# QData/FastSK

Measured on AMD Instinct MI355X. Metric: gkm kernel build: mismatch-combos/s, higher is better.
Workload: dtype u4 count planes (v_dot8_u32_u4), u32 register sums, u64 triangle (plain stores on the first pass over reset rows, else atomics); 1 GPU; config5: synthetic DNA 100000 x 300 bp, g=12 m=8 exact, 495 combos; n_seq=100000, seq_len=300, g=12, m=8, combos=495, parallelism=single GPU

## Files before the change

### fastsk_amd/csrc/fsk_engine_dense_shift.hip

```cpp
#include "fsk_engine_internal.h"
#include "fsk_kernels_dense_shift.h"

#include <map>

using namespace fsk_detail;

namespace fsk {

#define FSK_DMA_SHIFT 1
#define FSK_DMA_KERNEL k_dense_tile_shift
#define FSK_DMA_COMPACT 0
#include "fsk_tile_kernel_dma.inc"
#undef FSK_DMA_KERNEL
#undef FSK_DMA_COMPACT
#undef FSK_DMA_SHIFT

}

namespace fsk_detail {

bool dense_shift_plan(fsk_engine* e, const int32_t* combos, int n, u64 by_overflow, uint32_t max_chain) {
    ShiftPlan& p = e->shift;
    if (!(p.by_overflow == by_overflow && p.max_chain == max_chain && (int)p.combos.size() == n && std::equal(combos, combos + n, p.combos.begin()))) {
        p = ShiftPlan();
        p.combos.assign(combos, combos + n);
        p.by_overflow = by_overflow;
        p.max_chain = max_chain;
        const int k = e->k;
        std::map<std::vector<uint8_t>, std::vector<std::pair<int, int>>> shapes;
        for (int q = 0; q < n; ++q) {
            const uint8_t* pos = &e->all_pos[(size_t)combos[q] * k];
            std::vector<uint8_t> shape(pos, pos + k);
            for (auto& x : shape) x = (uint8_t)(x - pos[0]);
            shapes[shape].push_back({(int)pos[0], q});
        }
        std::vector<std::vector<int>> chains;
        for (auto& kv : shapes) {
            auto& v = kv.second;
            std::stable_sort(v.begin(), v.end(), [](const std::pair<int, int>& a, const std::pair<int, int>& b) { return a.first < b.first; });
            for (size_t i = 0; i < v.size(); ++i) {
                if (i == 0 || v[i].first != v[i - 1].first + 1 || (max_chain != 0u && chains.back().size() >= max_chain)) chains.emplace_back();
                chains.back().push_back(v[i].second);
            }
        }
        std::stable_sort(chains.begin(), chains.end(), [](const std::vector<int>& a, const std::vector<int>& b) { return a.size() > b.size(); });
        p.n_bases = (uint32_t)chains.size();
        p.order.resize((size_t)n);
        uint32_t derived = p.n_bases;
        size_t group_begin = 0;
        for (size_t c = 0; c < chains.size(); ++c) {
            const std::vector<int>& ch = chains[c];
            const uint32_t len = (uint32_t)ch.size();
            p.order[c] = ch[0];
            if (c == 0 || chains[c - 1].size() != ch.size() || (u64)(c - group_begin) >= by_overflow) {
                p.groups.push_back(0u);
                p.groups.push_back(len);
                group_begin = c;
            }
            p.groups[p.groups.size() - 2] = (uint32_t)c + 1u;
            uint32_t lower = (uint32_t)c;
            for (uint32_t u = 1; u < len; ++u) {
                const uint32_t upper = derived++;
                p.order[upper] = ch[u];
                p.steps.push_back(upper << 16 | lower);
                p.steps.push_back(len - u);
                p.wsum += len - u;
                lower = upper;
            }
        }
    }
    return !p.steps.empty() && n <= 32768 && ((u64)2 * e->maxW + 32) * p.wsum < ((u64)1 << 31);
}

int dense_shift_edge_keys(fsk_engine* e, const uint8_t* chunk_pos, uint32_t panels_pad) {
    ShiftPlan& p = e->shift;
    const uint32_t n_steps = (uint32_t)(p.steps.size() / 2), np_seq = panels_pad * fsk::PANEL;
    FSK_HIP(e->d_shift_steps.reserve(p.steps.size()));
    FSK_HIP(e->d_edge_keys.reserve((size_t)n_steps * np_seq));
    FSK_HIP(hipMemcpyAsync(e->d_shift_steps.p, p.steps.data(), p.steps.size() * sizeof(uint32_t), hipMemcpyHostToDevice, e->stream));
    FSK_LAUNCH(fsk::k_dense_edge_keys, dim3(panels_pad, (n_steps + 3u) / 4u), dim3(256), 0, e->stream, e->view(), e->cfg.g, e->k, e->sigma, chunk_pos,
               (const uint32_t*)e->d_shift_steps.p, n_steps, np_seq, e->d_edge_keys.p);
    FSK_HIP(hipStreamSynchronize(e->stream));
    e->st.launches += 1;
    return FSK_OK;
}

int dense_shift_keymajor(fsk_engine* e, uint32_t panels_pad, int nb, uint32_t Vq8) {
    const ShiftPlan& p = e->shift;
    e->shift_packed = false;
    if (e->tune.dense_shift_packed < 0 || p.max_chain != SHIFT_PACKED_CHAIN) return FSK_OK;
    const size_t plane = (size_t)panels_pad * Vq8 * fsk::PANEL * (size_t)nb;
    const size_t n_keys = (p.steps.size() / 2) * (size_t)panels_pad * fsk::PANEL;
    const size_t want = (2 * plane + n_keys) * sizeof(uint32_t);
    const char* why = nullptr;
    if (e->tune.dense_shift_plane_kb > 0 && want > (size_t)e->tune.dense_shift_plane_kb * 1024) why = "over the dense_shift_plane_kb cap";
    const size_t grow = (std::max(plane, e->d_KM.cap) - e->d_KM.cap + std::max(plane, e->d_KMH.cap) - e->d_KMH.cap +
                         std::max(n_keys, e->d_edge_offs.cap) - e->d_edge_offs.cap) * sizeof(uint32_t);
    if (!why && grow > 0) {
        size_t free_b = 0, total_b = 0;
        if (hipMemGetInfo(&free_b, &total_b) != hipSuccess) free_b = 0;
        if (grow > free_b / 2) why = "more than half of the free device memory";
        else if (e->d_KM.reserve(plane) != hipSuccess || e->d_KMH.reserve(plane) != hipSuccess || e->d_edge_offs.reserve(n_keys) != hipSuccess) {
            (void)hipGetLastError();
            e->d_KM.release(); e->d_KMH.release(); e->d_edge_offs.release();
            why = "hipMalloc failed";
        }
    }
    if (why) {
        if (e->trace())
            fprintf(stderr, "[fsk] dense shift classes: the key-major planes (%.1f MB) do not fit, %s: k_dense_shift_fix runs the corrections\n",
                    (double)want / 1e6, why);
        return FSK_OK;
    }
    const uint32_t n_pairs = panels_pad / 2u;
    const uint32_t kgrid = (uint32_t)(((size_t)n_pairs * nb * Vq8 * 16u + 255u) / 256u);
    FSK_LAUNCH(fsk::k_dense_keymajor, dim3(kgrid), dim3(256), 0, e->stream, (const uint32_t*)e->d_C4.p, n_pairs, nb, Vq8, e->d_KM.p);
    FSK_LAUNCH(fsk::k_dense_keymajor, dim3(kgrid), dim3(256), 0, e->stream, (const uint32_t*)e->d_C4H.p, n_pairs, nb, Vq8, e->d_KMH.p);
    FSK_LAUNCH(fsk::k_dense_edge_offs, dim3((uint32_t)((n_keys + 255u) / 256u)), dim3(256), 0, e->stream, (const uint16_t*)e->d_edge_keys.p, n_keys,
               e->d_edge_offs.p);
    e->st.launches += 3;
    e->shift_packed = true;
    return FSK_OK;
}

int dense_shift_tiles(fsk_engine* e, u64 n_tiles, int nb, uint32_t Vq8, uint32_t nst, u64* K, int store, uint32_t panels_pad) {
    const ShiftPlan& p = e->shift;
    int slot0 = 0;
    for (size_t gi = 0; gi + 1 < p.groups.size(); gi += 2) {
        const int end = (int)p.groups[gi];
        FSK_LAUNCH(fsk::k_dense_tile_shift, dim3((uint32_t)n_tiles, 1), dim3(256), 0, e->stream, (const uint32_t*)e->d_C4.p, (const uint32_t*)e->d_C4H.p,
                   (const uint32_t*)e->d_rowmask.p, (const uint32_t*)e->d_tiletab.p, nb, Vq8, nst, (uint32_t)e->N, K, end - slot0, gi == 0 ? store : 0,
                   slot0, p.groups[gi + 1]);
        slot0 = end;
    }
    if (e->shift_packed) {
        FSK_LAUNCH(fsk::k_dense_shift_packed, dim3((uint32_t)n_tiles), dim3(256), 0, e->stream, (const uint32_t*)e->d_KM.p, (const uint32_t*)e->d_KMH.p,
                   (const uint32_t*)e->d_rowmask.p, (const uint32_t*)e->d_tiletab.p, (const uint32_t*)e->d_shift_steps.p, (uint32_t)(p.steps.size() / 2),
                   (const uint32_t*)e->d_edge_offs.p, panels_pad * fsk::PANEL, nb, Vq8, p.n_bases, (uint32_t)(32u * p.wsum), (uint32_t)e->N, K);
    } else {
        FSK_LAUNCH(fsk::k_dense_shift_fix, dim3((uint32_t)n_tiles), dim3(512), 0, e->stream, (const uint32_t*)e->d_C4.p, (const uint32_t*)e->d_C4H.p,
                   (const uint32_t*)e->d_rowmask.p, (const uint32_t*)e->d_tiletab.p, (const uint32_t*)e->d_shift_steps.p, (uint32_t)(p.steps.size() / 2),
                   (const uint16_t*)e->d_edge_keys.p, panels_pad * fsk::PANEL, nb, Vq8, (uint32_t)e->N, K);
    }
    e->st.launches += (int32_t)(p.groups.size() / 2);
    return FSK_OK;
}

}
```

### fastsk_amd/csrc/fsk_engine_internal.h

```cpp
#pragma once
#include "fsk_common.h"

#include <algorithm>
#include <chrono>
#include <cmath>
#include <cstdarg>
#include <cstdio>
#include <cstdlib>
#include <cstring>
#include <string>
#include <array>
#include <atomic>
#include <thread>
#include <vector>

#include <cstdint>
#include <climits>

#include "../../include/fastsk_amd.h"
#include <condition_variable>
#include <functional>
#include <memory>
#include <mutex>

struct fsk_group;

namespace fsk_detail {

#define FSK_HIP(call)                                                                          \
    do {                                                                                       \
        hipError_t _e = (call);                                                                \
        if (_e != hipSuccess) return e->fail(FSK_EDEVICE, "%s failed: %s", #call, hipGetErrorString(_e)); \
    } while (0)

template <typename T>
struct DevBuf {
    T* p = nullptr;
    size_t cap = 0;
    hipError_t reserve(size_t n) {
        if (n <= cap) return hipSuccess;
        if (p) (void)hipFree(p);
        p = nullptr;
        cap = 0;
        hipError_t r = hipMalloc((void**)&p, n * sizeof(T));
        if (r == hipSuccess) cap = n;
        return r;
    }
    void release() {
        if (p) (void)hipFree(p);
        p = nullptr;
        cap = 0;
    }
};

struct DeviceScope {
    int prev = -1, dev;
    hipError_t err = hipSuccess;
    explicit DeviceScope(int d) : dev(d) {
        if (hipGetDevice(&prev) != hipSuccess) prev = -1;
        if (prev != dev) err = hipSetDevice(dev);
    }
    ~DeviceScope() {
        if (prev >= 0 && prev != dev) (void)hipSetDevice(prev);
    }
    DeviceScope(const DeviceScope&) = delete;
    DeviceScope& operator=(const DeviceScope&) = delete;
};
#define FSK_ON_DEVICE(e)                                                                      \
    DeviceScope fsk_on_device_((e)->cfg.device);                                             \
    if (fsk_on_device_.err != hipSuccess)                                                    \
        return (e)->fail(FSK_EDEVICE, "hipSetDevice(%d) failed: %s", (e)->cfg.device, hipGetErrorString(fsk_on_device_.err))

}

using fsk_detail::DevBuf;

#define FSK_TUNING_KEYS(X)                                                                                                          \
    X(trace, 0, 0, 1, "stderr: the tuning in force, where the host time of a load and of a variance-mode call goes")                 \
    X(profile, -1, -1, 2, "fsk_config.profile from here on (-1: as the engine was created)")                                          \
    X(compact, -1, -1, 1, "dense: key compaction off / on whatever the alphabet says (-1: a rare symbol decides)")                   \
    X(compact_rare, -1, -1, 1, "dense: keys that occur from the places of the rare symbols (1) or a marking pass over every window (0)") \
    X(tile_splits, 0, 0, 4096, "dense: combo splits per tile (0: by the size of the launch)")                                        \
    X(dense_small, 0, 0, 1, "dense: 1 = a split tile launch (small N) leaves its sums as 32-bit staging blocks that k_dense_widen adds into K (0: one 64-bit atomic a cell and split — measured faster: the atomics drain under other workgroups' dot products)")                                        \
    X(dense_shift, 0, -1, 1, "dense: one weighted Gram product per chain of shifted combinations, the other members by edge lookups (fsk_engine_dense_shift.hip) — 1 = whenever the call is eligible, -1 = never (0: when eligible, tile_splits = 0 and the launch has 16384 tiles or more, the size from which a tile has one workgroup anyway)") \
    X(dense_shift_packed, 0, -1, 0, "dense, shift classes: the derived steps from key-major planes, eight cells an LDS read (k_dense_keymajor, k_dense_shift_packed; chains cut at nine members) — 0 = whenever the shift path runs and the planes fit, -1 = never: k_dense_shift_fix on the count panels") \
    X(dense_shift_plane_kb, 0, 0, (int64_t)1 << 40, "dense, shift classes: the key-major planes and offsets may take this many KiB at most (0: half of the free memory; tests: the planes do not fit)") \
    X(dense_chunk, 0, 0, 1 << 24, "dense: cap of the count kernel's staging chunk, in windows (0: none)")                             \
    X(variance_dense_slots, 1, 0, 1, "variance mode, dense: 0 = zero fill + k_welford per iteration instead of storing slot triangles") \
    X(var_slots16, 1, 0, 1, "variance mode, sparse: 0 = u32 slot triangles from the start")                                          \
    X(sparse_global, 0, 0, 1, "sparse: every += as a 64-bit atomicAdd (k_sx_emit<DIRECT>) whatever N is")                             \
    X(sparse_unpacked, 0, 0, 1, "sparse: entries in the general 8 + 4 (+ 4) byte format whatever N is")                               \
    X(sparse_pairs, 1, 0, 1, "sparse: 0 = every update word 32 bits wide (1: unit products of clean runs travel two to a word)")      \
    X(sparse_sync, 0, 0, 1, "sparse: wait for every batch's word count and size its stream exactly")                                 \
    X(sparse_hint, 1, 0, 1, "sparse: 0 = the words per record of the previous set of sequences are never kept as a hint")             \
    X(sparse_exact_lanes, 0, 0, 2, "sparse: the batches of an exact accumulate never (1) / always (2) in two lanes (0: from six batches on)") \
    X(sparse_batch_records, 0, 0, (int64_t)1 << 31, "sparse: records per batch at most (0: 2^27)")                                   \
    X(guard_cap, 0, 0, (int64_t)1 << 40, "sparse: pretend the stream buffer holds this many words (0: its real size)")                \
    X(list_max_words, 0, 0, (int64_t)1 << 31, "sparse: update words of one batch beyond which its pairs go to K with atomics (0: 2^31)") \
    X(seg_scan_chunked, 0, 0, 1, "sparse: the three-launch segment scan whatever the tile count")                                    \
    X(extract_slots, 0, 0, 4, "sparse: slots per k_sx_extract_win workgroup, 1 or 4 (0: by the size of the launch)")                  \
    X(sparse_form, 0, 0, 3, "sparse: the update stage — 1 = owner bands whenever they exist, 2 = two-level blocks, 3 = 64-bit atomics (0: bands up to four LDS rounds a band, blocks beyond)") \
    X(blocks_sub_shift, 14, 4, 14, "sparse, blocks: log2 of the cells one k_sxb_consume workgroup sums in LDS (tests: small blocks on small inputs)") \
    X(blocks_max_bands, 512, 2, 512, "sparse, blocks: bands of one pass at most (tests: several passes on small inputs)")            \
    X(blocks_band_shift_max, 23, 4, 23, "sparse, blocks: log2 of a band's cells at most (tests)")                                    \
    X(blocks_pass_words, 0, 0, (int64_t)1 << 32, "sparse, blocks: update words of one pass at most (0: 2^31)")                       \
    X(sparse_desc, 0, -1, 1, "sparse, owner bands and two-level blocks: entries of many partners leave k_sx_emit as descriptors (one an entry; blocks: one per sub-band its partners fall into) that k_sx_consume / k_sxb_consume expand in LDS — 1 = always, -1 = never (0: once a batch of these sequences has shown sparse_desc_from pairs per record)") \
    X(sparse_desc_blocks, 1, 0, 1, "sparse, two-level blocks: 0 = never descriptors there (1: as sparse_desc says — one record per sub-band an entry's partners fall into)") \
    X(sparse_desc_cols, 1, 0, 3, "sparse, descriptors: where the partners are read from — 0 = the entries themselves; 1 = a column array (sequence id | multiplicity, 4 bytes) beside 8-byte entries, the entries themselves when they are packed (measured: 2-byte columns beside packed entries are no faster, 0.88 against 0.84 s in the large-g regime; 4-byte columns beside 8-byte entries 4.69 -> 4.44 ms a combo at N = 100k); tests: 2 = 4-byte columns always, 3 = 2-byte columns when N < 32768") \
    X(sparse_desc_min, 16, 1, 48, "sparse, descriptors: entries of more partners than this become descriptors (48: everything k_sx_emit does not bin in LDS; measured, large-g regime: 48 0.92 s, 32 0.85, 16 0.83-0.85, 8 0.88, 4 0.90)") \
    X(sparse_desc_from, 12, 1, 1 << 20, "sparse, descriptors: the pairs per sort record of a batch from which on the following batches use them (sparse_desc = 0)") \
    X(sparse_parts_target, 0, 0, 1 << 30, "sparse, owner bands: words of one k_sx_consume part (0: four LDS rounds' worth at least, 1/1024 of the batch's words; tests: several parts a band on small inputs)") \
    X(sparse_desc_parts, 2048, 1, 1 << 16, "sparse, descriptors: parts (k_sx_consume workgroups) the bands' streams are cut into, about") \
    X(sparse_share, 0, -1, 254, "sparse: leading kept positions sorted once per group of consecutive combos that share them (0: by cost; -1: never); batches of more than 16 slots only (smaller ones read their positions by id), and never when the presort's scratch passes a quarter of the free memory") \
    X(seed_splitmix, 0, 0, 1, "approx modes: 1 = fsk_set_seed draws the engine's older splitmix64 Fisher-Yates order (0: the reference's std::shuffle of minstd_rand0)") \
    X(mismatch_order, 0, 0, 1, "mismatch-weighted mode: 1 = the levels run from m = d down to 0 (0: from 0 up to d)")                   \
    X(collective, 0, 0, 2, "fsk_create_multi: FSK_COLL_* when fsk_config.collective is FSK_COLL_AUTO")                                \
    X(deadline_ms, 120000, -1, 86400000, "fsk_create_multi: the fail-fast bound when fsk_config.deadline_ms is 0 (negative: none)")   \
    X(svm_wg_max, 8192, 0, 8192, "fsk_svm_train: up to this many training rows the solver is one workgroup with alpha, G and y in LDS (k_svm_wg); beyond, two launches an iteration (k_svm_select_i / k_svm_select_j); 0 = always those") \
    X(svm_chunk, 256, 1, 65536, "fsk_svm_train: iterations enqueued between two reads of the solver's status record (k_svm_wg: iterations a launch)") \
    X(rows_tile, FSK_ROWS_TILE, FSK_ROWS_TILE, FSK_ROWS_TILE, "fsk_rows_build, read-only: the edge T of k_rows_syrk's tile of the rows kernel (compiled in)") \
    X(rows_panel, FSK_ROWS_PANEL, FSK_ROWS_PANEL, FSK_ROWS_PANEL, "fsk_rows_build, read-only: the consecutive train columns P a panel of k_rows_syrk stages in LDS (compiled in)") \
    FSK_TUNING_TEST_KEYS(X)
#ifdef FSK_TEST_HOOKS
#define FSK_TUNING_TEST_KEYS(X)                                            \
    X(fault_kind, 0, 0, 3, "test hook: 1 = host sleep, 2 = device spin before a band's collective; 3 = host sleep after the variance chains")   \
    X(fault_rank, -1, -1, 15, "test hook: the engine that is late")        \
    X(fault_band, -1, -1, 63, "test hook: before this band's collective")  \
    X(fault_ms, 0, 0, 60000, "test hook: by this many milliseconds")
#else
#define FSK_TUNING_TEST_KEYS(X)
#endif
struct fsk_tuning {
#define FSK_X(name, def, lo, hi, doc) int64_t name = (def);
    FSK_TUNING_KEYS(FSK_X)
#undef FSK_X
};

struct SxScratch {
    DevBuf<unsigned char> d_keys[2];
    DevBuf<uint32_t> d_blockhist, d_totals, d_tile_ent, d_ebase, d_Pk, d_Tk, d_ucount, d_uchunk, d_utot, d_list_off, d_ulist, d_part_base;
    DevBuf<u64> d_tile_stat;
    DevBuf<uint32_t> d_segc;
    DevBuf<int> d_tile_lrh, d_tile_rs, d_tile_lth, d_tile_ts;
    DevBuf<uint2> d_E;
    DevBuf<u64> d_sxstat;
    DevBuf<uint32_t> d_group_of, d_group_head, d_winp;
    DevBuf<unsigned char> d_part;
    DevBuf<uint32_t> d_ulist2, d_subcnt, d_suboff, d_subcur;
    DevBuf<uint32_t> d_dsubcnt, d_dsuboff, d_dsubcur;
    DevBuf<uint32_t> d_cols;
    void release() {
        d_ulist2.release(); d_subcnt.release(); d_suboff.release(); d_subcur.release();
        d_dsubcnt.release(); d_dsuboff.release(); d_dsubcur.release(); d_cols.release();
        d_group_of.release(); d_group_head.release(); d_winp.release(); d_part.release();
        for (auto& k : d_keys) k.release();
        d_blockhist.release(); d_totals.release(); d_tile_ent.release(); d_ebase.release(); d_Pk.release(); d_Tk.release();
        d_ucount.release(); d_uchunk.release(); d_utot.release(); d_list_off.release(); d_ulist.release(); d_part_base.release();
        d_tile_stat.release(); d_segc.release(); d_tile_lrh.release(); d_tile_rs.release(); d_tile_lth.release(); d_tile_ts.release();
        d_E.release(); d_sxstat.release();
    }
};

struct ShiftPlan {
    std::vector<int32_t> combos;
    u64 by_overflow = 0;
    std::vector<int32_t> order;
    std::vector<uint32_t> groups, steps;
    uint32_t n_bases = 0;
    uint32_t max_chain = 0;
    u64 wsum = 0;
};

struct SvmCvState {
    bool valid = false;
    std::vector<double> oof;
    std::vector<fsk_svm_cv_score> scores;
    std::vector<fsk_svm_cv_problem> problems;
    std::vector<double> alpha;
    std::vector<uint32_t> idx;
    std::vector<u64> st_off, idx_off;
    fsk_svm_cv_info info{};
    DevBuf<double> d_alpha, d_G, d_krow, d_coef, d_rho, d_oof;
    DevBuf<uint32_t> d_idx;
    DevBuf<int32_t> d_fold;
    DevBuf<signed char> d_y;
    DevBuf<unsigned char> d_prob, d_rec;
    void release() {
        d_alpha.release(); d_G.release(); d_krow.release(); d_coef.release(); d_rho.release(); d_oof.release();
        d_idx.release(); d_fold.release(); d_y.release(); d_prob.release(); d_rec.release();
    }
};

struct SvmState {
    bool valid = false;
    SvmCvState cv;
    std::vector<double> alpha;
    std::vector<signed char> y;
    double rho = 0;
    int kernel = 0;
    double w_pos = 1.0, w_neg = 1.0;
    double C = 0, eps = 0;
    int64_t max_iter = 0;
    SvmCvState cal;
    bool platt_valid = false;
    fsk_svm_platt_info platt{};
    fsk_svm_info info{};
    DevBuf<double> d_alpha, d_G, d_krow, d_coef, d_out;
    DevBuf<signed char> d_y;
    DevBuf<unsigned char> d_rec;
    void release() { d_alpha.release(); d_G.release(); d_krow.release(); d_coef.release(); d_out.release(); d_y.release(); d_rec.release(); cv.release(); cal.release(); }
    SvmState() = default;
    SvmState(const SvmState&) = delete;
    SvmState& operator=(const SvmState&) = delete;
    ~SvmState() { release(); }
};

struct RowsState {
    bool valid = false;
    DevBuf<double> d_L, d_diag;
    fsk_rows_info info{};
    void drop() { valid = false; d_L.release(); d_diag.release(); }
    RowsState() = default;
    RowsState(const RowsState&) = delete;
    RowsState& operator=(const RowsState&) = delete;
    ~RowsState() { drop(); }
};

struct fsk_engine {
    fsk_config cfg{};
    int cfg_profile0 = 0;
    fsk_tuning tune{};
    std::string err;
    int k = 0;
    int64_t ncomb = 0;
    hipStream_t stream = nullptr;
    hipEvent_t ev0 = nullptr, ev1 = nullptr;
    hipEvent_t ev_out = nullptr, ev_in = nullptr;
    fsk_group* group = nullptr;
    hipStream_t chain_stream = nullptr;
    int64_t lazy_lo = -1, lazy_hi = -1;
    bool store_next = false;
    uint32_t* h_stage = nullptr;
    size_t h_stage_cap = 0;
    bool stage_in_flight = false;
    double* h_prod = nullptr;
    size_t h_prod_cap = 0;

    bool loaded = false, finalized = false, result_f64 = false;
    int64_t N = 0, n_train = 0, n_test = 0, nfeat = 0, pairs = 0;
    uint32_t sigma = 0, Lmax = 0, Lmin = 0, maxW = 0, Vq = 0, n_panels = 0;
    int bits = 0;
    u64 V = 0;
    int path = 0;
    DevBuf<uint32_t> d_words, d_wstart, d_len, d_fstart, d_featseq;
    DevBuf<uint32_t> d_win;
    int win_words = 0;
    std::vector<uint32_t> h_len, h_fstart;
    bool featseq_ready = false;
    std::vector<int32_t> rc_tokens, rc_comps;
    bool revcomp = false;
    uint32_t maxW1 = 0;
    DevBuf<uint16_t> d_comp;
    std::vector<int32_t> wild_tokens;
    bool wild = false;
    DevBuf<uint32_t> d_vbits, d_vstart, d_fwin;
    std::vector<uint8_t> cw_profile;
    bool cw = false, fwin_on = false;
    uint32_t cw_n = 0;
    DevBuf<uint8_t> d_cw;

    std::vector<uint64_t> mm_c;
    std::vector<int64_t> mm_a;
    bool mm_plain = false;
    DevBuf<u64> mm_scratch;
    std::vector<int64_t> mm_ran_a;
    std::vector<int32_t> mm_ran_path;
    std::vector<double> mm_ran_level_ms, mm_ran_fold_ms;
    bool mm_on() const { return !mm_c.empty(); }

    std::vector<uint8_t> all_pos;
    DevBuf<uint8_t> d_pos, d_allpos;
    bool allpos_ready = false;
    std::vector<int32_t> order;
    bool order_set = false;
    uint64_t seed = 0;
    std::vector<double> stdevs;

    u64* d_K = nullptr;
    bool K_owned = false;
    int64_t bound_cells = 0;
    DevBuf<u64> K_store;
    DevBuf<double> d_Kf64, d_Khat, d_prod, d_diag, d_stage, d_bsum;
    DevBuf<unsigned char> d_seqblk;
    DevBuf<u64> d_stage_u64, d_Kslots;
    DevBuf<int64_t> d_cell_idx;

    DevBuf<uint32_t> d_C4, d_C4H, d_rowmask, d_flag;
    DevBuf<uint32_t> d_stage32;
    DevBuf<uint32_t> d_keybits;
    DevBuf<uint16_t> d_lut, d_vc;
    bool compact = false;
    bool compact_rare = false, rare_ready = false;
    uint32_t rare_mask = 0, rare_places = 0;
    DevBuf<u64> d_rare;
    DevBuf<uint32_t> d_rare_n, d_common;
    std::vector<uint16_t> h_vc_cache;
    double vc_sum = 0, vc_n = 0;
    DevBuf<uint32_t> d_tiletab;
    uint32_t tab_t0 = 0, tab_t1 = 0, tab_n = 0;
    uint32_t tab_ftt = 0xffffffffu;
    std::vector<int32_t> prep_combos;
    bool prep_valid = false, prep_overflow = false;
    bool prep_shift = false;
    uint32_t prep_chain = 0;
    ShiftPlan shift;
    DevBuf<uint32_t> d_shift_steps;
    DevBuf<uint16_t> d_edge_keys;
    DevBuf<uint32_t> d_KM, d_KMH, d_edge_offs;
    bool shift_packed = false;
    SxScratch sxs[2];
    hipStream_t lane_stream = nullptr;
    hipEvent_t ev_lane[4] = {nullptr, nullptr, nullptr, nullptr};
    DevBuf<uint32_t> d_owner_r0;
    DevBuf<u64> d_U;
    std::vector<uint32_t> h_owner_r0;
    uint32_t n_owners = 0, sx_rounds = 1, sx_cap = 0;
    uint32_t sx_rounds_slot = 1, sx_cap_slot = 0;
    int sx_pb = 16, sx_sb = 1, sx_keybits = 1, sx_own_shift = 13;
    int sx_symbits = 0;
    bool sx_lists = false, owner_ready = false;
    int n_cu = 256;
    int sx_form = 0;
    int sx_form_used = -1;
    u64 sx_passes = 0;
    int sx_share_used = 0;
    uint32_t sx_share_groups = 0;
    DevBuf<uint32_t> d_blk_r0;
    bool sx_pairs_asked = true;
    bool sx_pairs = false;
    int64_t owner_N = -1;
    DevBuf<u64> d_U2;
    std::vector<int32_t> u_combos;
    bool u_known = false, u_pending = false;
    u64 u_value = 0, u_extra = 0;
    unsigned char* h_sx_pos = nullptr;
    size_t h_sx_pos_cap = 0;
    u64* h_sx_stat = nullptr;
    size_t h_sx_stat_cap = 0;
    unsigned char* h_sx_head_pos = nullptr;
    u64* h_sx_head_stat = nullptr;
    bool sx_slot16 = false;
    bool sx_slot16_used = false;
    bool slots16_ok = true;
    uint32_t* h_sx_head_flag = nullptr;
    uint32_t* sx_ovf_now = nullptr;
    int sx_last_lane = 0;
    u64 sx_shape[4] = {0, 0, 0, 0};
    double sx_ppr = 0;
    bool sx_desc_used = false;
    double sx_wpr = 0;
    u64 sx_words_of(u64 nrec) const { return (u64)(sx_wpr * (double)nrec) + 1; }
    void sx_saw(u64 words, u64 nrec) { if (nrec) sx_wpr = std::max(sx_wpr, std::max(1e-9, (double)words / (double)nrec)); }
    bool sx_desc_now() const { return tune.sparse_desc > 0 || (tune.sparse_desc == 0 && sx_ppr >= (double)tune.sparse_desc_from); }
    void sx_saw_pairs(u64 pairs, u64 nrec) {
        if (!nrec) return;
        const bool was = sx_desc_now();
        sx_ppr = std::max(sx_ppr, (double)pairs / (double)nrec);
        if (!was && sx_desc_now()) sx_wpr = 0;
    }
    struct SxDefer { bool active = false; u64 cap = 0, nrec = 0; } sx_defer[8];
    u64 sx_redone = 0;
    bool sx_redoing = false;
    bool sx_exactly() const { return tune.sparse_sync != 0 || sx_redoing; }
    u64 sx_max_words() const { return tune.list_max_words > 0 ? std::min<u64>((u64)1 << 31, (u64)tune.list_max_words) : (u64)1 << 31; }
    bool trace() const { return tune.trace != 0; }

    fsk_stats st{};
    SvmState svm;
    RowsState rows;

    int fail(int code, const char* fmt, ...) {
        char buf[512];
        va_list ap;
        va_start(ap, fmt);
        vsnprintf(buf, sizeof buf, fmt, ap);
        va_end(ap);
        err = buf;
        return code;
    }
    fsk::SeqView view() const {
        return fsk::SeqView{d_words.p, d_wstart.p, d_len.p, (uint32_t)N, bits};
    }
    struct LazyTime { hipEvent_t a, b; double* acc; };
    std::vector<LazyTime> lazy_pending;
    std::vector<hipEvent_t> lazy_free;
    hipEvent_t lazy_open = nullptr;
    bool profile_sync() const { return cfg.profile == 1; }
    hipEvent_t lazy_event() {
        hipEvent_t ev = nullptr;
        if (!lazy_free.empty()) { ev = lazy_free.back(); lazy_free.pop_back(); }
        else if (hipEventCreate(&ev) != hipSuccess) ev = nullptr;
        return ev;
    }
    void harvest_times() {
        for (const LazyTime& t : lazy_pending) {
            float ms = 0;
            if (hipEventSynchronize(t.b) == hipSuccess && hipEventElapsedTime(&ms, t.a, t.b) == hipSuccess) *t.acc += ms;
            lazy_free.push_back(t.a);
            lazy_free.push_back(t.b);
        }
        lazy_pending.clear();
    }
    void harvest_finished() {
        size_t keep = 0;
        for (size_t i = 0; i < lazy_pending.size(); ++i) {
            const LazyTime t = lazy_pending[i];
            float ms = 0;
            if (hipEventQuery(t.b) == hipSuccess) {
                if (hipEventElapsedTime(&ms, t.a, t.b) == hipSuccess) *t.acc += ms;
                lazy_free.push_back(t.a);
                lazy_free.push_back(t.b);
            } else {
                (void)hipGetLastError();
                lazy_pending[keep++] = t;
            }
        }
        lazy_pending.resize(keep);
    }
    void lazy_interval(hipEvent_t a, hipEvent_t b, double* acc) {
        if (!a || !b) { if (a) lazy_free.push_back(a); if (b) lazy_free.push_back(b); return; }
        lazy_pending.push_back(LazyTime{a, b, acc});
        if (lazy_pending.size() >= 512 && lazy_pending.size() % 128 == 0) harvest_finished();
    }
    void tic(hipStream_t s = nullptr) {
        if (cfg.profile == 1) (void)hipEventRecord(ev0, s ? s : stream);
        else if (cfg.profile == 2) {
            if (lazy_open) lazy_free.push_back(lazy_open);
            lazy_open = lazy_event();
            if (lazy_open) (void)hipEventRecord(lazy_open, s ? s : stream);
        }
    }
    void toc(double* acc, hipStream_t s = nullptr) {
        if (cfg.profile == 1) {
            (void)hipEventRecord(ev1, s ? s : stream);
            (void)hipEventSynchronize(ev1);
            float ms = 0;
            (void)hipEventElapsedTime(&ms, ev0, ev1);
            *acc += ms;
        } else if (cfg.profile == 2 && lazy_open) {
            hipEvent_t b = lazy_event();
            if (b) (void)hipEventRecord(b, s ? s : stream);
            lazy_interval(lazy_open, b, acc);
            lazy_open = nullptr;
        }
    }
};

namespace fsk_detail {

constexpr size_t LDS_BUDGET = 150 * 1024;
constexpr u64 DENSE_MAX_KEYS = 16384;
constexpr size_t SPARSE_MAX_RECORDS = 1u << 27;
constexpr int FSK_RETRY_UNGROUPED = 1;

int tuning_set(fsk_tuning& t, const char* key, int64_t value, std::string& err);
int tuning_parse(fsk_tuning& t, const char* text, std::string& err);
std::string tuning_in_force(const fsk_tuning& t);
void set_create_error(const std::string& msg);
int64_t n_choose_k(int n, int k);
int materialise_zero(fsk_engine* e);
bool lazy_zero_possible(const fsk_engine* e);
int do_accumulate(fsk_engine* e, const int32_t* combos, int n, u64* K, int64_t row0 = 0, int64_t row1 = -1, u64 slot_stride = 0,
                  int defer = -1);
int make_diag(fsk_engine* e);
int launch_triangle(fsk_engine* e, u64 c0, u64 cnt, double* dst);
int rows_build(fsk_engine* e);
void default_order(fsk_engine* e);
void libstdcxx_shuffle_order(uint64_t seed, int64_t n, int32_t* out);

struct DensePlan { uint32_t CH = 0, Vcq = 0; size_t lds = 0; };
DensePlan dense_plan(uint32_t maxW, int g, uint32_t Vq, size_t extra = 0);
size_t dense_mode_lds(const fsk_engine* e);
int fetch_pending_u(fsk_engine* e);
int accumulate_dense(fsk_engine* e, const int32_t* combos, int n, u64* K, int64_t row0, int64_t row1);
size_t dense_small_stage_bytes(u64 n_tiles, int n_splits);
int dense_tile_small(fsk_engine* e, bool compact, u64 n_tiles, int n_splits, int nb, uint32_t Vq8, uint32_t nst, u64* K, int slots_per_split);

constexpr uint32_t SHIFT_PACKED_CHAIN = 9;
bool dense_shift_plan(fsk_engine* e, const int32_t* combos, int n, u64 by_overflow, uint32_t max_chain);
int dense_shift_edge_keys(fsk_engine* e, const uint8_t* chunk_pos, uint32_t panels_pad);
int dense_shift_keymajor(fsk_engine* e, uint32_t panels_pad, int nb, uint32_t Vq8);
int dense_shift_tiles(fsk_engine* e, u64 n_tiles, int nb, uint32_t Vq8, uint32_t nst, u64* K, int store, uint32_t panels_pad);

inline int sx_lane_of(const fsk_engine* e, int defer) { return (defer >= 0 && !e->profile_sync()) ? (defer & 1) : 0; }
struct SxPass { int64_t ra = 0, rb = 0; int t = 14, sub_shift = 14, pb = 8; uint32_t n_owners = 0, submax = 0, own_base = 0; std::vector<uint32_t> r0; };
bool blocks_plan_pass(fsk_engine* e, int64_t ra, int64_t rb, SxPass* out);
void plan_owner_bands(fsk_engine* e);
bool sx_harvest(fsk_engine* e, int slot);
int accumulate_sparse(fsk_engine* e, const int32_t* combos, int n, u64* K, int64_t row0, int64_t row1, u64 slot_stride = 0,
                      int defer = -1);

int run_variance_mode(fsk_engine* e, int T, int chain_first = 0, int chain_step = 1);

int one_load_sequences(fsk_engine* e, const int32_t* tokens, const int64_t* offsets, int64_t n_train, int64_t n_test);
int one_reset_counts(fsk_engine* e);
int one_reset_counts_rows(fsk_engine* e, int64_t row_begin, int64_t row_end);
int one_accumulate_rows(fsk_engine* e, const int32_t* combos, int32_t n, int64_t row_begin, int64_t row_end);
int one_synchronize(fsk_engine* e);
int one_finalize(fsk_engine* e);
int one_set_combo_order(fsk_engine* e, const int32_t* order, int32_t n);
int one_set_complement(fsk_engine* e, const int32_t* tokens, const int32_t* complements, int32_t n);
int one_set_wildcards(fsk_engine* e, const int32_t* tokens, int32_t n);
int one_set_center_weights(fsk_engine* e, const uint32_t* w, int32_t n);
int one_get_stats(fsk_engine* e, fsk_stats* out);
void one_destroy(fsk_engine* e);
void skip_variance_combos(fsk_engine* e, std::vector<int32_t>& used);
int approx_chains(const fsk_engine* e);
int mismatch_solve(int g, const uint64_t* c, int n, std::vector<int64_t>& a, std::string& why);
int mismatch_compute(fsk_engine* e, const int32_t* tokens, const int64_t* offsets, int64_t n_train, int64_t n_test);

int group_load_sequences(fsk_engine* e, const int32_t* tokens, const int64_t* offsets, int64_t n_train, int64_t n_test);
int group_reset_counts(fsk_engine* e, int64_t row_begin, int64_t row_end);
int group_accumulate(fsk_engine* e, const int32_t* combos, int32_t n);
int group_synchronize(fsk_engine* e);
int group_finalize(fsk_engine* e);
int group_compute(fsk_engine* e, const int32_t* tokens, const int64_t* offsets, int64_t n_train, int64_t n_test);
int group_set_combo_order(fsk_engine* e, const int32_t* order, int32_t n);
int group_set_seed(fsk_engine* e, uint64_t seed);
int group_set_complement(fsk_engine* e, const int32_t* tokens, const int32_t* complements, int32_t n);
int group_set_wildcards(fsk_engine* e, const int32_t* tokens, int32_t n);
int group_set_center_weights(fsk_engine* e, const uint32_t* w, int32_t n);
int group_get_stats(fsk_engine* e, fsk_stats* out);
int group_set_skip_test_block(fsk_engine* e, int32_t skip);
int group_set_tuning(fsk_engine* e, const char* key, int64_t value, std::string& err);
void group_set_profile(fsk_engine* e, int profile);
void group_destroy(fsk_engine* e);
void group_note_bound_counts(fsk_engine* e);

}
```

### fastsk_amd/csrc/fsk_kernels_dense_shift.h

```cpp
#pragma once
#include "fsk_bytesel.h"
#include "fsk_common.h"

namespace fsk {

__device__ __forceinline__ uint32_t panel_seq(uint32_t p) { return (p >> 2) + 16u * (p & 3u); }

__global__ __launch_bounds__(256) void k_dense_edge_keys(SeqView S, int g, int k, uint32_t sigma, const uint8_t* combo_pos, const uint32_t* steps,
                                                         uint32_t n_steps, uint32_t np_seq, uint16_t* keys) {
    const uint32_t r = threadIdx.x & 63u, step = blockIdx.y * 4u + (threadIdx.x >> 6), panel = blockIdx.x;
    if (step >= n_steps) return;
    const uint32_t seq = panel * PANEL + r;
    const uint32_t sl = steps[2u * step], up = sl >> 16, lo = sl & 0xffffu;
    uint32_t kd = 0, ks = 0;
    if (seq < S.n_seq) {
        const uint32_t len = S.len[seq], wbase = S.wstart[seq];
        if (len >= (uint32_t)g) {
            const uint32_t last = len - (uint32_t)g;
            for (int c = 0; c < k; ++c) {
                kd = kd * sigma + fetch_sym(S.words, wbase, (uint32_t)combo_pos[(size_t)lo * k + c], S.bits);
                ks = ks * sigma + fetch_sym(S.words, wbase, last + (uint32_t)combo_pos[(size_t)up * k + c], S.bits);
            }
        }
    }
    keys[(size_t)step * np_seq + panel * PANEL + panel_slot(r)] = (uint16_t)(kd | (ks << 8));
}

__global__ __launch_bounds__(512, 4) void k_dense_shift_fix(const uint32_t* C4, const uint32_t* C4H, const uint32_t* rowmask, const uint32_t* tile_tab,
                                                            const uint32_t* steps, uint32_t n_steps, const uint16_t* keys, uint32_t np_seq,
                                                            int n_slots, uint32_t Vq8, uint32_t N, u64* K) {
    constexpr int ROWS = 32;
    constexpr int HALF = ROWS * PANEL;
    constexpr int PBUF = 4 * HALF;
    constexpr int QW = 16;
    __shared__ __attribute__((aligned(1024))) uint32_t P[2 * PBUF];
    const uint32_t tid = threadIdx.x, lane = tid & 63u;
    const uint32_t w = (uint32_t)__builtin_amdgcn_readfirstlane(tid >> 6);
    const uint32_t tile = tile_tab[blockIdx.x];
    const uint32_t ti = tile >> 16, tj = tile & 0xffffu;
    const size_t slot_stride = (size_t)Vq8 * PANEL;
    const size_t panel_stride = (size_t)n_slots * slot_stride;

    int accR[2][QW], accC[2][QW];
#pragma unroll
    for (int h = 0; h < 2; ++h)
#pragma unroll
        for (int q = 0; q < QW; ++q) accR[h][q] = accC[h][q] = 0;

    const fsk_hw::lds_addr_t lds_wave = fsk_hw::lds_address(P) + w * 1024u;
    auto load_stage = [&](const uint32_t* plane, int buf, uint32_t sl) {
        const uint32_t up = sl >> 16, lo = sl & 0xffffu;
#pragma unroll
        for (int q = 0; q < 4; ++q) {
            const uint32_t panel = (q < 2 ? ti : tj) * 2u + (uint32_t)(q & 1);
            const uint32_t* src = plane + panel * panel_stride + (size_t)(q < 2 ? up : lo) * slot_stride;
            fsk_hw::panel_rows_to_lds(src, Vq8 * PANEL * 4u, lds_wave + (uint32_t)(buf * PBUF + q * HALF) * 4u, tid * 16u);
        }
    };
    auto load_meta = [&](uint32_t s, uint32_t sl, uint32_t& kA, uint32_t& kB, uint32_t& fl) {
        const uint16_t* ks = keys + (size_t)s * np_seq;
        kA = (uint32_t)ks[ti * TILE + lane] | (uint32_t)ks[ti * TILE + PANEL + lane] << 16;
        kB = (uint32_t)ks[tj * TILE + lane] | (uint32_t)ks[tj * TILE + PANEL + lane] << 16;
        const uint32_t up = sl >> 16, lo = sl & 0xffffu;
        const uint32_t mA = rowmask[(size_t)(ti * 2u) * n_slots + up] | rowmask[(size_t)(ti * 2u + 1u) * n_slots + up];
        const uint32_t mB = rowmask[(size_t)(tj * 2u) * n_slots + lo] | rowmask[(size_t)(tj * 2u + 1u) * n_slots + lo];
        fl = mA | mB;
    };
    auto edge = [&](const uint32_t* p0, size_t stride, uint32_t kk, int mul, int& a0, int& a1) {
        const uint32_t kd = kk & 255u, ks = (kk >> 8) & 255u;
        const uint32_t* rd = p0 + (kd >> 3) * PANEL + lane;
        const uint32_t* rs = p0 + (ks >> 3) * PANEL + lane;
        const uint32_t shd = (kd & 7u) * 4u, shs = (ks & 7u) * 4u;
        a0 += ((int)((rs[0] >> shs) & 15u) - (int)((rd[0] >> shd) & 15u)) * mul;
        a1 += ((int)((rs[stride] >> shs) & 15u) - (int)((rd[stride] >> shd) & 15u)) * mul;
    };

    uint32_t sl_cur = steps[0], wt_cur = steps[1];
    uint32_t sl_nxt = n_steps > 1u ? steps[2] : 0u, wt_nxt = n_steps > 1u ? steps[3] : 0u;
    uint32_t kA_n, kB_n, fl_n;
    load_meta(0u, sl_cur, kA_n, kB_n, fl_n);
    uint32_t sl_n2 = 0u, wt_n2 = 0u;
    int buf = 0;
    load_stage(C4, 0, (uint32_t)__builtin_amdgcn_readfirstlane(fsk_hw::vgpr_copy(sl_cur)));
    fsk_hw::wait_panel_rows();
    __syncthreads();
    const uint32_t lsel = (w & 3u) * (uint32_t)QW, hsh = (w >> 2) * 16u;
    for (uint32_t s = 0; s < n_steps; ++s) {
        const uint32_t kA = fsk_hw::vgpr_copy(kA_n), kB = fsk_hw::vgpr_copy(kB_n);
        const uint32_t fl = (uint32_t)__builtin_amdgcn_readfirstlane(fsk_hw::vgpr_copy(fl_n));
        const uint32_t sl = (uint32_t)__builtin_amdgcn_readfirstlane(fsk_hw::vgpr_copy(sl_cur));
        const int wt = (int)((uint32_t)__builtin_amdgcn_readfirstlane(fsk_hw::vgpr_copy(wt_cur)) & 255u);
        if (s + 1u < n_steps) {
            const uint32_t sn = (uint32_t)__builtin_amdgcn_readfirstlane(fsk_hw::vgpr_copy(sl_nxt));
            if (s + 2u < n_steps) {
                sl_n2 = steps[2u * (s + 2u)];
                wt_n2 = steps[2u * (s + 2u) + 1u];
            }
            load_meta(s + 1u, sn, kA_n, kB_n, fl_n);
            load_stage(C4, buf ^ 1, sn);
        }
        const uint32_t* pb = P + buf * PBUF;
        auto lookups = [&](int mul) {
#pragma unroll
            for (int q = 0; q < QW; ++q) {
                const uint32_t kk = (fsk_hw::readlane(kB, lsel + (uint32_t)q) >> hsh) & 0xffffu;
                edge(pb, (size_t)HALF, kk, mul, accR[0][q], accR[1][q]);
                if ((q & 3) == 3) asm volatile("" ::: "memory");
            }
#pragma unroll
            for (int q = 0; q < QW; ++q) {
                const uint32_t kk = (fsk_hw::readlane(kA, lsel + (uint32_t)q) >> hsh) & 0xffffu;
                edge(pb + 2 * HALF, (size_t)HALF, kk, mul, accC[0][q], accC[1][q]);
                if ((q & 3) == 3) asm volatile("" ::: "memory");
            }
        };
        lookups(wt);
        if (fl != 0u) {
            __syncthreads();
            load_stage(C4H, buf, sl);
            fsk_hw::wait_panel_rows();
            __syncthreads();
            lookups(16 * wt);
        }
        fsk_hw::wait_panel_rows();
        __syncthreads();
        sl_cur = sl_nxt; wt_cur = wt_nxt;
        sl_nxt = sl_n2; wt_nxt = wt_n2;
        buf ^= 1;
    }
    int* const T = reinterpret_cast<int*>(P);
#pragma unroll
    for (int h = 0; h < 2; ++h)
#pragma unroll
        for (int q = 0; q < QW; ++q) {
            const uint32_t i = (uint32_t)h * PANEL + lane, j = w * (uint32_t)QW + (uint32_t)q;
            T[i * TILE + ((j + i) & (TILE - 1u))] = accR[h][q];
        }
    __syncthreads();
#pragma unroll
    for (int h = 0; h < 2; ++h) {
        const uint32_t jd = (uint32_t)h * PANEL + lane;
        const u64 j = (u64)tj * TILE + (uint32_t)h * PANEL + panel_seq(lane);
#pragma unroll
        for (int q = 0; q < QW; ++q) {
            const uint32_t id = w * (uint32_t)QW + (uint32_t)q;
            const u64 i = (u64)ti * TILE + (id >> 6) * PANEL + panel_seq(id & 63u);
            const int v = accC[h][q] + T[id * TILE + ((jd + id) & (TILE - 1u))];
            if (i < N && j <= i && v != 0) atomicAdd(&K[tri_index(i, j)], (u64)(long long)v);
        }
    }
}

__device__ __forceinline__ uint32_t km_swizzle(uint32_t key) { return ((key >> 1) & 3u) << 2; }
__device__ __forceinline__ uint32_t km_offset(uint32_t key) { return key << 6 | km_swizzle(key) << 2; }

__global__ __launch_bounds__(256) void k_dense_keymajor(const uint32_t* plane, uint32_t n_pairs, int n_slots, uint32_t Vq8, uint32_t* KM) {
    const size_t id = (size_t)blockIdx.x * 256u + threadIdx.x;
    const uint32_t t = (uint32_t)id & 15u;
    size_t rest = id >> 4;
    const uint32_t row = (uint32_t)(rest % Vq8);
    rest /= Vq8;
    const uint32_t slot = (uint32_t)(rest % (uint32_t)n_slots);
    const size_t pair = rest / (uint32_t)n_slots;
    if (pair >= n_pairs) return;
    const size_t slot_stride = (size_t)Vq8 * PANEL, panel_stride = (size_t)n_slots * slot_stride;
    const uint32_t* src = plane + 2u * pair * panel_stride + slot * slot_stride + (size_t)row * PANEL + 4u * t;
    const uint4 a = *reinterpret_cast<const uint4*>(src), b = *reinterpret_cast<const uint4*>(src + panel_stride);
    const uint32_t in[8] = {a.x, a.y, a.z, a.w, b.x, b.y, b.z, b.w};
    uint32_t* out = KM + (pair * (size_t)n_slots + slot) * ((size_t)Vq8 * 128u);
#pragma unroll
    for (uint32_t q = 0; q < 8u; ++q) {
        uint32_t v = 0;
#pragma unroll
        for (uint32_t n = 0; n < 8u; ++n) v |= ((in[n] >> (4u * q)) & 15u) << (4u * n);
        const uint32_t key = row * 8u + q;
        out[key * 16u + (t ^ km_swizzle(key))] = v;
    }
}

__global__ __launch_bounds__(256) void k_dense_edge_offs(const uint16_t* keys, size_t n, uint32_t* offs) {
    const size_t q = (size_t)blockIdx.x * 256u + threadIdx.x;
    if (q >= n) return;
    const uint32_t kk = keys[q];
    offs[q] = km_offset(kk & 255u) | km_offset(kk >> 8) << 16;
}

__global__ __launch_bounds__(256, 2) void k_dense_shift_packed(const uint32_t* KM, const uint32_t* KMH, const uint32_t* rowmask, const uint32_t* tile_tab,
                                                               const uint32_t* steps, uint32_t n_steps, const uint32_t* offs, uint32_t np_seq,
                                                               int n_slots, uint32_t Vq8, uint32_t n_bases, uint32_t bias, uint32_t N, u64* K) {
    constexpr uint32_t SIDE = 256u * 16u;
    constexpr uint32_t PBUF = 2u * SIDE;
    __shared__ __attribute__((aligned(1024))) uint32_t P[2 * PBUF];
    const uint32_t tid = threadIdx.x, lane = tid & 63u;
    const uint32_t w = (uint32_t)__builtin_amdgcn_readfirstlane(tid >> 6);
    const uint32_t M4 = (uint32_t)__builtin_amdgcn_readfirstlane(fsk_hw::vgpr_copy(0x0f0f0f0fu)), B4 = fsk_hw::vgpr_copy(0x10101010u);
    const uint32_t tr = (w >> 1) * 8u + (lane >> 3), tc = (w & 1u) * 8u + (lane & 7u);
    const uint32_t tile = tile_tab[blockIdx.x];
    const uint32_t ti = tile >> 16, tj = tile & 0xffffu;
    const size_t slot_stride = (size_t)Vq8 * 128u;
    const size_t pair_stride = (size_t)n_slots * slot_stride;
    const uint32_t side_bytes = Vq8 * 512u;

    uint32_t acc[8][8], Rr[2][8], Rc[2][8];
#pragma unroll
    for (int a = 0; a < 8; ++a) {
#pragma unroll
        for (int b = 0; b < 8; ++b) acc[a][b] = 0u;
        Rr[0][a] = Rr[1][a] = Rc[0][a] = Rc[1][a] = 0u;
    }

    const fsk_hw::lds_addr_t lds_wave = fsk_hw::lds_address(P) + w * 1024u;
    auto load_stage = [&](const uint32_t* plane, uint32_t buf, uint32_t sl) {
        const uint32_t up = sl >> 16, lo = sl & 0xffffu;
#pragma unroll
        for (uint32_t side = 0; side < 2u; ++side) {
            const uint32_t* src = plane + (side == 0u ? ti : tj) * pair_stride + (size_t)(side == 0u ? up : lo) * slot_stride;
#pragma unroll
            for (uint32_t q = 0; q < 4u; ++q)
                if (q * 4096u < side_bytes)
                    fsk_hw::panel_rows_to_lds(src, side_bytes, lds_wave + (buf * PBUF + side * SIDE + q * 1024u) * 4u, q * 4096u + tid * 16u);
        }
    };
    auto load_offs = [&](uint32_t s, uint4 (&oR)[2], uint4 (&oC)[2]) {
        const uint32_t* os = offs + (size_t)s * np_seq;
#pragma unroll
        for (uint32_t h = 0; h < 2u; ++h) {
            oR[h] = *reinterpret_cast<const uint4*>(os + ti * TILE + h * PANEL + 4u * tr);
            oC[h] = *reinterpret_cast<const uint4*>(os + tj * TILE + h * PANEL + 4u * tc);
        }
    };
    auto flagged = [&](uint32_t sl) {
        const uint32_t up = sl >> 16, lo = sl & 0xffffu;
        const uint32_t mA = rowmask[(size_t)(ti * 2u) * n_slots + up] | rowmask[(size_t)(ti * 2u + 1u) * n_slots + up];
        const uint32_t mB = rowmask[(size_t)(tj * 2u) * n_slots + lo] | rowmask[(size_t)(tj * 2u + 1u) * n_slots + lo];
        return mA | mB;
    };
    auto lds_at = [&](uint32_t byte_off) { return *reinterpret_cast<const uint32_t*>(reinterpret_cast<const char*>(P) + byte_off); };

    uint32_t sl = steps[0], wt = steps[1] & 255u, fl = flagged(sl);
    uint32_t sn = n_steps > 1u ? steps[2] : 0u, wn = n_steps > 1u ? steps[3] : 0u;
    uint4 oR_n[2], oC_n[2];
    load_offs(0u, oR_n, oC_n);
    uint32_t buf = 0;
    load_stage(KM, 0u, sl);
    fsk_hw::wait_panel_rows();
    __syncthreads();
    for (uint32_t s = 0; s < n_steps; ++s) {
        uint32_t oR[8], oC[8];
#pragma unroll
        for (int h = 0; h < 2; ++h) {
            oR[4 * h] = fsk_hw::vgpr_copy(oR_n[h].x); oR[4 * h + 1] = fsk_hw::vgpr_copy(oR_n[h].y);
            oR[4 * h + 2] = fsk_hw::vgpr_copy(oR_n[h].z); oR[4 * h + 3] = fsk_hw::vgpr_copy(oR_n[h].w);
            oC[4 * h] = fsk_hw::vgpr_copy(oC_n[h].x); oC[4 * h + 1] = fsk_hw::vgpr_copy(oC_n[h].y);
            oC[4 * h + 2] = fsk_hw::vgpr_copy(oC_n[h].z); oC[4 * h + 3] = fsk_hw::vgpr_copy(oC_n[h].w);
        }
        if (s + 1u < n_steps) {
            load_offs(s + 1u, oR_n, oC_n);
            load_stage(KM, buf ^ 1u, sn);
        }
        if ((sl & 0xffffu) < n_bases) {
#pragma unroll
            for (int a = 0; a < 8; ++a) Rr[0][a] = Rr[1][a] = Rc[0][a] = Rc[1][a] = 0u;
        }
        const uint32_t baseA = buf * PBUF * 4u, baseB = baseA + SIDE * 4u;
        const uint32_t xA = (tr * 4u) | baseA, xB = (tc * 4u) | baseB;
        uint32_t dA[8], sA[8], dB[8], sB[8];
        auto read_A = [&](int e) { dA[e] = lds_at(fsk_hw::xor_word<0>(oC[e], xA)); sA[e] = lds_at(fsk_hw::xor_word<1>(oC[e], xA)); };
        auto read_B = [&](int e) { dB[e] = lds_at(fsk_hw::xor_word<0>(oR[e], xB)); sB[e] = lds_at(fsk_hw::xor_word<1>(oR[e], xB)); };
        auto row_term = [&](int e) {
            Rr[0][e] += ((sA[e] & M4) | B4) - (dA[e] & M4);
            Rr[1][e] += (((sA[e] >> 4) & M4) | B4) - ((dA[e] >> 4) & M4);
            acc[0][e] = fsk_hw::add_byte<0>(acc[0][e], Rr[0][e]); acc[1][e] = fsk_hw::add_byte<0>(acc[1][e], Rr[1][e]);
            acc[2][e] = fsk_hw::add_byte<1>(acc[2][e], Rr[0][e]); acc[3][e] = fsk_hw::add_byte<1>(acc[3][e], Rr[1][e]);
            acc[4][e] = fsk_hw::add_byte<2>(acc[4][e], Rr[0][e]); acc[5][e] = fsk_hw::add_byte<2>(acc[5][e], Rr[1][e]);
            acc[6][e] = fsk_hw::add_byte<3>(acc[6][e], Rr[0][e]); acc[7][e] = fsk_hw::add_byte<3>(acc[7][e], Rr[1][e]);
        };
        auto col_term = [&](int e) {
            Rc[0][e] += ((sB[e] & M4) | B4) - (dB[e] & M4);
            Rc[1][e] += (((sB[e] >> 4) & M4) | B4) - ((dB[e] >> 4) & M4);
            acc[e][0] = fsk_hw::add_byte<0>(acc[e][0], Rc[0][e]); acc[e][1] = fsk_hw::add_byte<0>(acc[e][1], Rc[1][e]);
            acc[e][2] = fsk_hw::add_byte<1>(acc[e][2], Rc[0][e]); acc[e][3] = fsk_hw::add_byte<1>(acc[e][3], Rc[1][e]);
            acc[e][4] = fsk_hw::add_byte<2>(acc[e][4], Rc[0][e]); acc[e][5] = fsk_hw::add_byte<2>(acc[e][5], Rc[1][e]);
            acc[e][6] = fsk_hw::add_byte<3>(acc[e][6], Rc[0][e]); acc[e][7] = fsk_hw::add_byte<3>(acc[e][7], Rc[1][e]);
        };
#pragma unroll
        for (int e = 0; e < 8; ++e) read_A(e);
        fsk_hw::first_use(dA[0], sA[0], dA[1], sA[1], dA[2], sA[2], dA[3], sA[3]);
#pragma unroll
        for (int e = 0; e < 4; ++e) read_B(e);
#pragma unroll
        for (int e = 0; e < 4; ++e) row_term(e);
        fsk_hw::first_use(dA[4], sA[4], dA[5], sA[5], dA[6], sA[6], dA[7], sA[7]);
#pragma unroll
        for (int e = 4; e < 8; ++e) read_B(e);
#pragma unroll
        for (int e = 4; e < 8; ++e) row_term(e);
        fsk_hw::first_use(dB[0], sB[0], dB[1], sB[1], dB[2], sB[2], dB[3], sB[3]);
#pragma unroll
        for (int e = 0; e < 4; ++e) col_term(e);
        fsk_hw::first_use(dB[4], sB[4], dB[5], sB[5], dB[6], sB[6], dB[7], sB[7]);
#pragma unroll
        for (int e = 4; e < 8; ++e) col_term(e);
        if (fl != 0u) {
            __syncthreads();
            load_stage(KMH, buf, sl);
            fsk_hw::wait_panel_rows();
            __syncthreads();
            const uint32_t mul = 16u * wt;
#pragma unroll
            for (int e = 0; e < 8; ++e) {
                read_A(e);
                read_B(e);
#pragma unroll
                for (int n = 0; n < 8; ++n) {
                    acc[n][e] += (((sA[e] >> (4 * n)) & 15u) - ((dA[e] >> (4 * n)) & 15u)) * mul;
                    acc[e][n] += (((sB[e] >> (4 * n)) & 15u) - ((dB[e] >> (4 * n)) & 15u)) * mul;
                }
            }
        }
        uint32_t fl_n = 0u, sl_n2 = 0u, wt_n2 = 0u;
        if (s + 1u < n_steps) {
            fl_n = flagged(sn);
            if (s + 2u < n_steps) {
                sl_n2 = steps[2u * (s + 2u)];
                wt_n2 = steps[2u * (s + 2u) + 1u];
            }
        }
        fsk_hw::wait_panel_rows();
        __syncthreads();
        sl = sn; wt = wn & 255u; fl = fl_n;
        sn = sl_n2; wn = wt_n2;
        buf ^= 1u;
    }
#pragma unroll
    for (int er = 0; er < 8; ++er) {
        const u64 i = (u64)ti * TILE + tile_index(tr, (uint32_t)er);
#pragma unroll
        for (int ec = 0; ec < 8; ++ec) {
            const u64 j = (u64)tj * TILE + tile_index(tc, (uint32_t)ec);
            const int v = (int)(acc[er][ec] - bias);
            if (i < N && j <= i && v != 0) atomicAdd(&K[tri_index(i, j)], (u64)(long long)v);
        }
    }
}

}
```

Before: 419.8 combos/s.

## Update shifted key-major planes in LDS instead of restaging each chain step

Adds an in-place mode to k_dense_shift_packed, enabled by default through a new tuning knob. For derived chain steps whose tile has no flagged counts above 15, the kernel no longer stages the next step's planes from global memory. Instead it edits the current LDS buffer with two LDS atomics per sequence, adding one nibble and subtracting another at the edge offsets. This saves global loads and LDS fills per step, at the cost of an extra barrier, LDS atomics and a deeper step-lookahead pipeline.

```diff
diff --git a/fastsk_amd/csrc/fsk_engine_dense_shift.hip b/fastsk_amd/csrc/fsk_engine_dense_shift.hip
--- a/fastsk_amd/csrc/fsk_engine_dense_shift.hip
+++ b/fastsk_amd/csrc/fsk_engine_dense_shift.hip
@@ -134,7 +134,8 @@
         slot0 = end;
     }
     if (e->shift_packed) {
-        FSK_LAUNCH(fsk::k_dense_shift_packed, dim3((uint32_t)n_tiles), dim3(256), 0, e->stream, (const uint32_t*)e->d_KM.p, (const uint32_t*)e->d_KMH.p,
+        const auto k_packed = e->tune.dense_shift_inplace != 0 ? fsk::k_dense_shift_packed<true> : fsk::k_dense_shift_packed<false>;
+        FSK_LAUNCH(k_packed, dim3((uint32_t)n_tiles), dim3(256), 0, e->stream, (const uint32_t*)e->d_KM.p, (const uint32_t*)e->d_KMH.p,
                    (const uint32_t*)e->d_rowmask.p, (const uint32_t*)e->d_tiletab.p, (const uint32_t*)e->d_shift_steps.p, (uint32_t)(p.steps.size() / 2),
                    (const uint32_t*)e->d_edge_offs.p, panels_pad * fsk::PANEL, nb, Vq8, p.n_bases, (uint32_t)(32u * p.wsum), (uint32_t)e->N, K);
     } else {
diff --git a/fastsk_amd/csrc/fsk_engine_internal.h b/fastsk_amd/csrc/fsk_engine_internal.h
--- a/fastsk_amd/csrc/fsk_engine_internal.h
+++ b/fastsk_amd/csrc/fsk_engine_internal.h
@@ -84,6 +84,7 @@
     X(dense_small, 0, 0, 1, "dense: 1 = a split tile launch (small N) leaves its sums as 32-bit staging blocks that k_dense_widen adds into K (0: one 64-bit atomic a cell and split — measured faster: the atomics drain under other workgroups' dot products)")                                        \
     X(dense_shift, 0, -1, 1, "dense: one weighted Gram product per chain of shifted combinations, the other members by edge lookups (fsk_engine_dense_shift.hip) — 1 = whenever the call is eligible, -1 = never (0: when eligible, tile_splits = 0 and the launch has 16384 tiles or more, the size from which a tile has one workgroup anyway)") \
     X(dense_shift_packed, 0, -1, 0, "dense, shift classes: the derived steps from key-major planes, eight cells an LDS read (k_dense_keymajor, k_dense_shift_packed; chains cut at nine members) — 0 = whenever the shift path runs and the planes fit, -1 = never: k_dense_shift_fix on the count panels") \
+    X(dense_shift_inplace, 1, 0, 1, "dense, shift classes: k_dense_shift_packed stages a chain's first planes and makes every further step's in LDS, one nibble up and one down a sequence (a step that meets a count above 15 in its tile, and the step behind it, are staged) — 0 = every step staged") \
     X(dense_shift_plane_kb, 0, 0, (int64_t)1 << 40, "dense, shift classes: the key-major planes and offsets may take this many KiB at most (0: half of the free memory; tests: the planes do not fit)") \
     X(dense_chunk, 0, 0, 1 << 24, "dense: cap of the count kernel's staging chunk, in windows (0: none)")                             \
     X(variance_dense_slots, 1, 0, 1, "variance mode, dense: 0 = zero fill + k_welford per iteration instead of storing slot triangles") \
diff --git a/fastsk_amd/csrc/fsk_kernels_dense_shift.h b/fastsk_amd/csrc/fsk_kernels_dense_shift.h
--- a/fastsk_amd/csrc/fsk_kernels_dense_shift.h
+++ b/fastsk_amd/csrc/fsk_kernels_dense_shift.h
@@ -185,6 +185,7 @@
     offs[q] = km_offset(kk & 255u) | km_offset(kk >> 8) << 16;
 }
 
+template <bool INPLACE>
 __global__ __launch_bounds__(256, 2) void k_dense_shift_packed(const uint32_t* KM, const uint32_t* KMH, const uint32_t* rowmask, const uint32_t* tile_tab,
                                                                const uint32_t* steps, uint32_t n_steps, const uint32_t* offs, uint32_t np_seq,
                                                                int n_slots, uint32_t Vq8, uint32_t n_bases, uint32_t bias, uint32_t N, u64* K) {
@@ -239,6 +240,11 @@
 
     uint32_t sl = steps[0], wt = steps[1] & 255u, fl = flagged(sl);
     uint32_t sn = n_steps > 1u ? steps[2] : 0u, wn = n_steps > 1u ? steps[3] : 0u;
+    uint32_t s2 = 0u, w2 = 0u, fl_nx = 0u;
+    if constexpr (INPLACE) {
+        if (n_steps > 2u) { s2 = steps[4]; w2 = steps[5]; }
+        if (n_steps > 1u) fl_nx = flagged(sn);
+    }
     uint4 oR_n[2], oC_n[2];
     load_offs(0u, oR_n, oC_n);
     uint32_t buf = 0;
@@ -254,9 +260,12 @@
             oC[4 * h] = fsk_hw::vgpr_copy(oC_n[h].x); oC[4 * h + 1] = fsk_hw::vgpr_copy(oC_n[h].y);
             oC[4 * h + 2] = fsk_hw::vgpr_copy(oC_n[h].z); oC[4 * h + 3] = fsk_hw::vgpr_copy(oC_n[h].w);
         }
+        const bool same = INPLACE && s + 1u < n_steps && (sn & 0xffffu) >= n_bases && fl == 0u && fl_nx == 0u;
+        uint32_t uo_n = 0u;
         if (s + 1u < n_steps) {
             load_offs(s + 1u, oR_n, oC_n);
-            load_stage(KM, buf ^ 1u, sn);
+            if (same) uo_n = offs[(size_t)(w < 2u ? s + 1u : s) * np_seq + (w < 2u ? ti : tj) * TILE + (tid & 127u)];
+            else load_stage(KM, buf ^ 1u, sn);
         }
         if ((sl & 0xffffu) < n_bases) {
 #pragma unroll
@@ -319,7 +328,15 @@
             }
         }
         uint32_t fl_n = 0u, sl_n2 = 0u, wt_n2 = 0u;
-        if (s + 1u < n_steps) {
+        if constexpr (INPLACE) {
+            if (s + 2u < n_steps) {
+                fl_n = flagged(s2);
+                if (s + 3u < n_steps) {
+                    sl_n2 = steps[2u * (s + 3u)];
+                    wt_n2 = steps[2u * (s + 3u) + 1u];
+                }
+            }
+        } else if (s + 1u < n_steps) {
             fl_n = flagged(sn);
             if (s + 2u < n_steps) {
                 sl_n2 = steps[2u * (s + 2u)];
@@ -328,9 +345,26 @@
         }
         fsk_hw::wait_panel_rows();
         __syncthreads();
-        sl = sn; wt = wn & 255u; fl = fl_n;
-        sn = sl_n2; wn = wt_n2;
-        buf ^= 1u;
+        if (same) {
+            const uint32_t uo = fsk_hw::vgpr_copy(uo_n), od = uo & 0xffffu, os = uo >> 16;
+            if (od != os) {
+                const uint32_t p = tid & 127u, t4 = p & 0x3cu, e = (p >> 6) * 4u + (p & 3u);
+                const uint32_t base = buf * PBUF + (w >> 1) * SIDE, inc = 1u << (4u * e);
+                atomicAdd(&P[base + ((os ^ t4) >> 2)], inc);
+                atomicAdd(&P[base + ((od ^ t4) >> 2)], 0u - inc);
+            }
+            __syncthreads();
+        } else {
+            buf ^= 1u;
+        }
+        if constexpr (INPLACE) {
+            sl = sn; wt = wn & 255u; fl = fl_nx;
+            sn = s2; wn = w2; fl_nx = fl_n;
+            s2 = sl_n2; w2 = wt_n2;
+        } else {
+            sl = sn; wt = wn & 255u; fl = fl_n;
+            sn = sl_n2; wn = wt_n2;
+        }
     }
 #pragma unroll
     for (int er = 0; er < 8; ++er) {
```

Result: faster. 436.1 combos/s (median of 6 runs) (+3.9%).
